# Stansfash/nonstationary-precip

Hardware: AMD Instinct MI355X
Metric: dsvi_elbo_steps_per_sec (higher is better)
Workload: dtype f32; 1 GPU; 2-layer DSVI DeepGP (hidden 3->2 + last 2->1), M=1024, S=10, minibatch 4096 (global, split over the GPUs) of synthetic N=1e5 spatio-temporal grid; fwd+ELBO+bwd+Adam; M=1024, S=10, per_gpu_batch=4096, global_batch=4096, N=100000, parallelism=dp1, kzz_cholesky_dtype=f64, hipgraph=True

## Files before the change

### nonstationary-precip_amd/csrc/gemm_i8.hip

```cpp
#include <cstdlib>
#include "common.h"

namespace {

#ifndef NSGP_I8_DMA
#define NSGP_I8_DMA 1
#endif
constexpr int I8_BM = 128, I8_BN = 64, I8_BK = 32;
constexpr int I8_SW = 5;

typedef int v4i __attribute__((ext_vector_type(4)));
typedef int v16i __attribute__((ext_vector_type(16)));

__global__ __launch_bounds__(256) void i8_slice_w_kernel(const double* __restrict__ W, int64_t M, int64_t Mp, int64_t KB,
                                                         signed char* __restrict__ Wd, double* __restrict__ wsc) {
    __shared__ double lds[4];
    const int64_t b = blockIdx.y, m = blockIdx.x;
    signed char* out = Wd + b * (int64_t)I8_SW * KB * 2 * Mp * 16;
    const int64_t plane = KB * 2 * Mp * 16;
    if (m >= M) {
        for (int64_t k = threadIdx.x; k < KB * 32; k += 256)
            for (int a = 0; a < I8_SW; ++a) out[a * plane + ((k >> 5) * 2 + ((k >> 4) & 1)) * Mp * 16 + m * 16 + (k & 15)] = 0;
        return;
    }
    const double* row = W + (b * M + m) * M;
    const auto nmax = [](double a, double c) { return (a > c || a != a) ? a : c; };
    double mx = 0.0;
    for (int64_t k = threadIdx.x; k <= m; k += 256) mx = nmax(fabs(row[k]), mx);
    for (int off = 32; off > 0; off >>= 1) mx = nmax(__shfl_xor(mx, off, 64), mx);
    if ((threadIdx.x & 63) == 0) lds[threadIdx.x >> 6] = mx;
    __syncthreads();
    mx = nmax(nmax(lds[0], lds[1]), nmax(lds[2], lds[3]));
    const bool fin = mx <= 1.7976931348623157e308;
    int e = 0;
    (void)frexp(fin ? mx : 0.0, &e);
    const double rs = (fin && mx > 0.0) ? ldexp(1.0, e) : 1.0;
    if (threadIdx.x == 0) wsc[b * M + m] = fin ? rs / 64.0 : __builtin_nan("");
    const double inv = 64.0 / rs;
    for (int64_t k = threadIdx.x; k < KB * 32; k += 256) {
        double t = (fin && k <= m && k < M) ? row[k] * inv : 0.0;
        const int64_t o = ((k >> 5) * 2 + ((k >> 4) & 1)) * Mp * 16 + m * 16 + (k & 15);
#pragma unroll
        for (int a = 0; a < I8_SW; ++a) {
            const double d = rint(t);
            out[a * plane + o] = (signed char)(int)d;
            t = (t - d) * 128.0;
        }
    }
}

template <int D, int SK>
__global__ __launch_bounds__(256) void i8_rbf_build_kernel(const float* __restrict__ Z, const float* __restrict__ x, int64_t sx,
                                                           const float* __restrict__ ls, const float* __restrict__ os,
                                                           int64_t M, int64_t n, int64_t np, int64_t KB,
                                                           signed char* __restrict__ Kd, double* __restrict__ ksc,
                                                           float* __restrict__ Kf) {
    const int64_t b = blockIdx.z, kb = blockIdx.y;
    const int64_t j = (int64_t)blockIdx.x * 256 + threadIdx.x;
    __shared__ double zs[32][D];
    __shared__ int bad;
    if (threadIdx.x == 0) bad = 0;
    if (threadIdx.x < 32 * D) {
        const int kk = threadIdx.x / D, d = threadIdx.x % D;
        const int64_t k = kb * 32 + kk;
        zs[kk][d] = k < M ? (double)Z[(b * M + k) * D + d] / (double)ls[b * D + d] : 0.0;
    }
    __syncthreads();
    const double osd = (double)os[b];
    bool fin = fabs(osd) <= 1.7976931348623157e308;
#pragma unroll
    for (int d = 0; d < D; ++d) fin = fin && fabs((double)ls[b * D + d]) <= 1.7976931348623157e308;
    int e = 0;
    (void)frexp(fin ? osd : 0.0, &e);
    const double cs = ldexp(1.0, e);
    const double sc = fin ? osd * 64.0 / cs : 0.0;
    if (j < np) {
        double xs[D];
#pragma unroll
        for (int d = 0; d < D; ++d) xs[d] = j < n ? (double)x[b * sx + j * D + d] / (double)ls[b * D + d] : 0.0;
        signed char* out = Kd + b * (int64_t)SK * KB * 2 * np * 16;
        const int64_t plane = KB * 2 * np * 16;
#pragma unroll
        for (int h = 0; h < 2; ++h) {
            int pk[SK][4] = {};
#pragma unroll
            for (int q = 0; q < 16; ++q) {
                const int kk = h * 16 + q;
                double r2 = 0.0;
#pragma unroll
                for (int d = 0; d < D; ++d) { const double df = zs[kk][d] - xs[d]; r2 = __builtin_fma(df, df, r2); }
                const bool in = j < n && kb * 32 + kk < M;
                const bool nan_e = in && r2 != r2;
                if (nan_e) bad = 1;
                const double ev = in ? t_fexp<double>(-0.5 * r2) : 0.0;
                const double evd = nan_e ? 0.0 : ev;
                if (Kf && in) Kf[(b * M + kb * 32 + kk) * n + j] = (float)(osd * ev);
                double t = sc * evd;
#pragma unroll
                for (int s = 0; s < SK; ++s) {
                    const double dg = rint(t);
                    pk[s][q >> 2] |= ((int)dg & 0xFF) << (8 * (q & 3));
                    t = (t - dg) * 128.0;
                }
            }
#pragma unroll
            for (int s = 0; s < SK; ++s) {
                v4i v = {pk[s][0], pk[s][1], pk[s][2], pk[s][3]};
                *reinterpret_cast<v4i*>(out + s * plane + (kb * 2 + h) * np * 16 + j * 16) = v;
            }
        }
    }
    __syncthreads();
    if (threadIdx.x == 0)
        ksc[(b * KB + kb) * gridDim.x + blockIdx.x] = (fin && !bad) ? cs / 64.0 : __builtin_nan("");
}

template <int P64, int SK, int LEV>
__global__ __launch_bounds__(256, 2) void i8_proj_kernel(const signed char* __restrict__ Wd, const double* __restrict__ wsc,
                                                         const signed char* __restrict__ Kd, const double* __restrict__ ksc,
                                                         const float* __restrict__ rv, int64_t M, int64_t n, int64_t Mp,
                                                         int64_t np, int64_t KB, int tiles_n, float* __restrict__ Y,
                                                         void* __restrict__ p0, void* __restrict__ p1, int part_rows) {
    extern __shared__ __attribute__((aligned(16))) unsigned char i8_smem[];
    constexpr int A_STAGE = I8_SW * 2 * I8_BM * 16, B_STAGE = SK * 2 * I8_BN * 16;
    unsigned char* As = i8_smem;
    unsigned char* Bs = i8_smem + 2 * A_STAGE;
    const int tid = threadIdx.x, lane = tid & 63, wave = __builtin_amdgcn_readfirstlane(tid >> 6);
    const int wm0 = (wave >> 1) * 64, wn0 = (wave & 1) * 32;
    const int64_t bb = blockIdx.y;
    const int tiles_m = (int)(Mp / I8_BM);
    const int bm = tiles_m - 1 - (int)blockIdx.x / tiles_n;
    const int bn = (int)blockIdx.x % tiles_n;
    const int64_t m0 = (int64_t)bm * I8_BM, n0 = (int64_t)bn * I8_BN;
    int nkb = (int)((m0 + I8_BM) / I8_BK);
    if (nkb > KB) nkb = (int)KB;
    const signed char* Wb = Wd + bb * (int64_t)I8_SW * KB * 2 * Mp * 16;
    const signed char* Kb = Kd + bb * (int64_t)SK * KB * 2 * np * 16;
    const int64_t wplane = KB * 2 * Mp * 16, kplane = KB * 2 * np * 16;

    const signed char* ga[5];
#pragma unroll
    for (int j = 0; j < 5; ++j) {
        const int q = tid + 256 * j;
        const int a = q >> 8, h = (q >> 7) & 1, row = q & 127;
        ga[j] = Wb + a * wplane + (int64_t)h * Mp * 16 + (m0 + row) * 16;
    }
    constexpr int NPB = (SK * 128 + 255) / 256;
    const signed char* gb[NPB];
#pragma unroll
    for (int j = 0; j < NPB; ++j) {
        int q = tid + 256 * j;
        if (q >= SK * 128) q = SK * 128 - 1;
        const int s = q >> 7, h = (q >> 6) & 1, col = q & 63;
        gb[j] = Kb + s * kplane + (int64_t)h * np * 16 + (n0 + col) * 16;
    }
    const int64_t astep = 2 * Mp * 16, bstep = 2 * np * 16;
#if NSGP_I8_DMA
    typedef const __attribute__((address_space(1))) void* gptr_t;
    typedef __attribute__((address_space(3))) void* lptr_t;
    auto dma = [&](int kb, int buf) __attribute__((always_inline)) {
#pragma unroll
        for (int j = 0; j < 5; ++j)
            __builtin_amdgcn_global_load_lds((gptr_t)(ga[j] + (int64_t)kb * astep),
                                             (lptr_t)(As + buf * A_STAGE + (wave * 64 + 256 * j) * 16), 16, 0, 0);
#pragma unroll
        for (int j = 0; j < NPB; ++j)
            if (wave * 64 + 256 * j < SK * 128)
                __builtin_amdgcn_global_load_lds((gptr_t)(gb[j] + (int64_t)kb * bstep),
                                                 (lptr_t)(Bs + buf * B_STAGE + (wave * 64 + 256 * j) * 16), 16, 0, 0);
    };
#endif
    v4i ra[5], rb[NPB];
    auto gload = [&](int kb) __attribute__((always_inline)) {
#pragma unroll
        for (int j = 0; j < 5; ++j) ra[j] = *reinterpret_cast<const v4i*>(ga[j] + (int64_t)kb * astep);
#pragma unroll
        for (int j = 0; j < NPB; ++j) rb[j] = *reinterpret_cast<const v4i*>(gb[j] + (int64_t)kb * bstep);
    };
    auto sstore = [&](int buf) __attribute__((always_inline)) {
#pragma unroll
        for (int j = 0; j < 5; ++j) *reinterpret_cast<v4i*>(As + buf * A_STAGE + (tid + 256 * j) * 16) = ra[j];
#pragma unroll
        for (int j = 0; j < NPB; ++j)
            if (tid + 256 * j < SK * 128) *reinterpret_cast<v4i*>(Bs + buf * B_STAGE + (tid + 256 * j) * 16) = rb[j];
    };

    v16i acc[LEV][2];
#pragma unroll
    for (int l = 0; l < LEV; ++l)
#pragma unroll
        for (int i = 0; i < 2; ++i)
#pragma unroll
            for (int r = 0; r < 16; ++r) acc[l][i][r] = 0;

    const int wave_nkb = __builtin_amdgcn_readfirstlane((int)((m0 + wm0 + 64 + I8_BK - 1) / I8_BK));
    const int half = lane >> 5, lr = lane & 31;
#if NSGP_I8_DMA
    dma(0, 0);
    asm volatile("s_waitcnt vmcnt(0)" ::: "memory");
#else
    gload(0);
    sstore(0);
#endif
    __syncthreads();
    for (int kb = 0; kb < nkb; ++kb) {
        const int buf = kb & 1;
#if NSGP_I8_DMA
        if (kb + 1 < nkb) dma(kb + 1, buf ^ 1);
#else
        if (kb + 1 < nkb) gload(kb + 1);
#endif
        if (kb < wave_nkb) {
            v4i af[2][2], bf[SK];
#pragma unroll
            for (int s = 0; s < SK; ++s)
                bf[s] = *reinterpret_cast<const v4i*>(Bs + buf * B_STAGE + ((s * 2 + half) * I8_BN + wn0 + lr) * 16);
#pragma unroll
            for (int i = 0; i < 2; ++i)
                af[0][i] = *reinterpret_cast<const v4i*>(As + buf * A_STAGE + ((0 * 2 + half) * I8_BM + wm0 + 32 * i + lr) * 16);
#pragma unroll
            for (int a = 0; a < I8_SW; ++a) {
                if (a + 1 < I8_SW) {
#pragma unroll
                    for (int i = 0; i < 2; ++i)
                        af[(a + 1) & 1][i] = *reinterpret_cast<const v4i*>(
                            As + buf * A_STAGE + (((a + 1) * 2 + half) * I8_BM + wm0 + 32 * i + lr) * 16);
                }
#pragma unroll
                for (int s = 0; s < SK; ++s)
                    if (a + s < LEV) {
#pragma unroll
                        for (int i = 0; i < 2; ++i)
                            acc[a + s][i] = __builtin_amdgcn_mfma_i32_32x32x32_i8(af[a & 1][i], bf[s], acc[a + s][i], 0, 0, 0);
                    }
            }
        }
#if NSGP_I8_DMA
        asm volatile("s_waitcnt vmcnt(0)" ::: "memory");
#else
        if (kb + 1 < nkb) sstore(buf ^ 1);
#endif
        __syncthreads();
    }

    const int64_t gx = (np + 255) >> 8;
    const double* ks = ksc + bb * KB * gx + (n0 >> 8);
    const double kslot = tid < nkb ? ks[(int64_t)tid * gx] : 0.0;
    const double kscale = __syncthreads_or(kslot != kslot) ? __builtin_nan("") : ks[0];
    double sdot = 0.0, ssq = 0.0;
    const int64_t col = n0 + wn0 + lr;
    const float* rvb = rv ? rv + bb * M : nullptr;
#pragma unroll
    for (int i = 0; i < 2; ++i)
#pragma unroll
        for (int r = 0; r < 16; ++r) {
            const int64_t row = m0 + wm0 + 32 * i + (r & 3) + 8 * (r >> 2) + 4 * half;
            double v = (double)acc[LEV - 1][i][r];
#pragma unroll
            for (int l = LEV - 2; l >= 0; --l) v = __builtin_fma(v, 0.0078125, (double)acc[l][i][r]);
            const bool in = row < M && col < n;
            v *= (in ? wsc[bb * M + row] : 0.0) * kscale;
            if (in) Y[(bb * M + row) * n + col] = (float)v;
            sdot += v * ((rvb && in) ? (double)rvb[row] : 0.0);
            ssq += v * v;
        }
    sdot += __shfl_xor(sdot, 32, 64);
    ssq += __shfl_xor(ssq, 32, 64);
    double* red = reinterpret_cast<double*>(i8_smem);
    __syncthreads();
    if (lane < 32) {
        red[(0 + (wave >> 1)) * I8_BN + wn0 + lane] = sdot;
        red[(2 + (wave >> 1)) * I8_BN + wn0 + lane] = ssq;
    }
    __syncthreads();
    if (tid < I8_BN && n0 + tid < n) {
        const int64_t o = (bb * part_rows + bm) * n + n0 + tid;
        const double d = red[tid] + red[I8_BN + tid], q = red[2 * I8_BN + tid] + red[3 * I8_BN + tid];
        if (P64) {
            if (p0) reinterpret_cast<double*>(p0)[o] = d;
            reinterpret_cast<double*>(p1)[o] = q;
        } else {
            if (p0) reinterpret_cast<float*>(p0)[o] = (float)d;
            reinterpret_cast<float*>(p1)[o] = (float)q;
        }
    }
}

static inline int64_t i8_mp(int64_t M) { return cdiv64(M, I8_BM) * I8_BM; }
static inline int64_t i8_np(int64_t n) { return cdiv64(n, I8_BN) * I8_BN; }
static inline int64_t i8_kb(int64_t M) { return cdiv64(M, I8_BK); }

}

extern "C" {

int nsgp_i8_supported(int64_t M) { return (M >= 1 && M <= 4096) ? 1 : 0; }
size_t nsgp_i8_w_planes_bytes(int64_t batch, int64_t M) {
    return (batch > 0 && M > 0) ? (size_t)(batch * I8_SW * i8_kb(M) * 2 * i8_mp(M) * 16) : 0;
}
size_t nsgp_i8_k_planes_bytes(int64_t batch, int64_t M, int64_t n, int planes) {
    return (batch > 0 && M > 0 && n > 0 && (planes == 4 || planes == 5)) ? (size_t)(batch * planes * i8_kb(M) * 2 * i8_np(n) * 16) : 0;
}
size_t nsgp_i8_tiles(int64_t M) { return M > 0 ? (size_t)cdiv64(M, I8_BM) : 0; }
size_t nsgp_i8_kscale_count(int64_t batch, int64_t M, int64_t n) {
    return (batch > 0 && M > 0 && n > 0) ? (size_t)(batch * i8_kb(M) * cdiv64(i8_np(n), 256)) : 0;
}

int nsgp_i8_slice_w_f64(const double* W, int64_t batch, int64_t M, void* Wd, double* wscale, void* stream) {
    if (!W) return -1; if (batch < 0) return -2; if (M < 0 || !nsgp_i8_supported(M > 0 ? M : 1)) return -3;
    if (!Wd) return -4; if (!wscale) return -5;
    if (batch == 0 || M == 0) return 0;
    if (batch > 65535) return -2;
    hipLaunchKernelGGL(i8_slice_w_kernel, dim3((unsigned)i8_mp(M), (unsigned)batch), dim3(256), 0, (hipStream_t)stream, W, M,
                       i8_mp(M), i8_kb(M), (signed char*)Wd, wscale);
    return nsgp_launch_status();
}

int nsgp_i8_rbf_build_f32(const float* Z, const float* x, int64_t x_batch_stride, const float* ls, const float* os,
                          int64_t batch, int64_t M, int64_t n, int D, int planes, void* Kd, double* kscale, float* Kzx_f32,
                          void* stream) {
    if (planes != 4 && planes != 5) return -10;
    if (!Z) return -1; if (!x) return -2; if (x_batch_stride < 0) return -3; if (!ls) return -4; if (!os) return -5;
    if (batch < 0) return -6; if (M < 0 || !nsgp_i8_supported(M > 0 ? M : 1)) return -7; if (n < 0) return -8;
    if (D < 1 || D > 4) return -9; if (!Kd) return -10; if (!kscale) return -11;
    if (batch == 0 || M == 0 || n == 0) return 0;
    if (batch > 65535 || i8_kb(M) > 65535) return -6;
    const int64_t np = i8_np(n), KB = i8_kb(M);
    dim3 grid((unsigned)cdiv64(np, 256), (unsigned)KB, (unsigned)batch);
    hipStream_t st = (hipStream_t)stream;
    signed char* kd = (signed char*)Kd;
#define NSGP_I8_BUILD(DD, SS) hipLaunchKernelGGL((i8_rbf_build_kernel<DD, SS>), grid, dim3(256), 0, st, Z, x, x_batch_stride, ls, os, M, n, np, KB, kd, kscale, Kzx_f32)
    if (planes == 4) {
        switch (D) { case 1: NSGP_I8_BUILD(1, 4); break; case 2: NSGP_I8_BUILD(2, 4); break; case 3: NSGP_I8_BUILD(3, 4); break;
                     default: NSGP_I8_BUILD(4, 4); break; }
    } else {
        switch (D) { case 1: NSGP_I8_BUILD(1, 5); break; case 2: NSGP_I8_BUILD(2, 5); break; case 3: NSGP_I8_BUILD(3, 5); break;
                     default: NSGP_I8_BUILD(4, 5); break; }
    }
#undef NSGP_I8_BUILD
    return nsgp_launch_status();
}

int nsgp_svgp_tri_gemm_colstats_i8(const void* Wd, const double* wscale, const void* Kd, const double* kscale,
                                   int planes, const float* rowvec, int64_t batch, int64_t M, int64_t n, float* Y,
                                   void* part_dot, void* part_sq, int64_t part_rows, int partials_f64, void* stream) {
    if (planes != 4 && planes != 5) return -5;
    if (!Wd) return -1; if (!wscale) return -2; if (!Kd) return -3; if (!kscale) return -4;
    if (batch < 0) return -6; if (M < 0 || !nsgp_i8_supported(M > 0 ? M : 1)) return -7; if (n < 0) return -8;
    if (!Y) return -9; if (!part_sq) return -11; if (part_rows < cdiv64(M > 0 ? M : 1, I8_BM)) return -12;
    if (batch == 0 || M == 0 || n == 0) return 0;
    const int64_t Mp = i8_mp(M), np = i8_np(n), KB = i8_kb(M);
    const int64_t tiles_n = np / I8_BN, tiles = (Mp / I8_BM) * tiles_n;
    if (tiles > 2147483647LL || batch > 65535) return -8;
    const size_t lds = 2 * (size_t)(I8_SW * 2 * I8_BM * 16 + planes * 2 * I8_BN * 16);
    hipStream_t st = (hipStream_t)stream;
    dim3 grid((unsigned)tiles, (unsigned)batch);
#define NSGP_I8_PROJ(PP, SS) hipLaunchKernelGGL((i8_proj_kernel<PP, SS, (SS == 5 ? 6 : 5)>), grid, dim3(256), lds, st, (const signed char*)Wd, wscale, \
        (const signed char*)Kd, kscale, rowvec, M, n, Mp, np, KB, (int)tiles_n, Y, part_dot, part_sq, (int)part_rows)
    if (planes == 4) { if (partials_f64) NSGP_I8_PROJ(1, 4); else NSGP_I8_PROJ(0, 4); }
    else { if (partials_f64) NSGP_I8_PROJ(1, 5); else NSGP_I8_PROJ(0, 5); }
#undef NSGP_I8_PROJ
    return nsgp_launch_status();
}

}
```

Baseline: 233.4 steps/s.

## Add persistent triple-buffered i8 projection kernel with wider tiles

Adds a persistent kernel for the triangular int8 projection GEMM. It launches one block per CU, walks tiles in a serpentine order starting from the heaviest triangular rows, doubles the N tile to 128 with 512 threads, and triple-buffers global-to-LDS DMA loads across tile boundaries. The aim is to cut launch and tail imbalance on the triangular workload and to overlap loads with MFMA. The old path stays reachable through an environment variable. It uses more LDS per block, and the occupancy and schedule are more complex.

```diff
diff --git a/nonstationary-precip_amd/csrc/gemm_i8.hip b/nonstationary-precip_amd/csrc/gemm_i8.hip
--- a/nonstationary-precip_amd/csrc/gemm_i8.hip
+++ b/nonstationary-precip_amd/csrc/gemm_i8.hip
@@ -1,3 +1,4 @@
+#include <atomic>
 #include <cstdlib>
 #include "common.h"
 
@@ -286,9 +287,188 @@
     }
 }
 
+template <int P64, int SK, int LEV>
+__global__ __launch_bounds__(512, 2) void i8_proj_persistent_kernel(
+        const signed char* __restrict__ Wd, const double* __restrict__ wsc, const signed char* __restrict__ Kd,
+        const double* __restrict__ ksc, const float* __restrict__ rv, int64_t M, int64_t n, int64_t Mp, int64_t np,
+        int64_t KB, int tiles_m, int tiles_n, int batch, float* __restrict__ Y, void* __restrict__ p0, void* __restrict__ p1,
+        int part_rows) {
+    extern __shared__ __attribute__((aligned(16))) unsigned char i8_smem[];
+    constexpr int BN = 2 * I8_BN;
+    constexpr int NL = 20 + 4 * SK;
+    constexpr int STAGE = NL * 1024;
+    constexpr int NJ = (NL + 7) / 8;
+    constexpr int NMIN = NL / 8;
+    double* red = reinterpret_cast<double*>(i8_smem + 3 * STAGE);
+    const int tid = threadIdx.x, lane = tid & 63, wave = __builtin_amdgcn_readfirstlane(tid >> 6);
+    const int wr = wave >> 2, wm0 = wr * 64, wn0 = (wave & 3) * 32;
+    const int half = lane >> 5, lr = lane & 31;
+    const int G = (int)gridDim.x, w = (int)blockIdx.x;
+    const int per_row = tiles_n * batch, T = tiles_m * per_row;
+    const int64_t wplane = KB * 2 * Mp * 16, kplane = KB * 2 * np * 16;
+    const int64_t astep = 2 * Mp * 16, bstep = 2 * np * 16;
+
+    const auto entry = [&](int r) { return r * G + ((r & 1) ? G - 1 - w : w); };
+    struct Tile { int bm, bb, bn, nkb; };
+    const auto tile_of = [&](int i) {
+        Tile t;
+        t.bm = tiles_m - 1 - i / per_row;
+        const int rem = i % per_row;
+        t.bb = rem / tiles_n;
+        t.bn = rem % tiles_n;
+        t.nkb = (int)((((int64_t)t.bm + 1) * I8_BM) / I8_BK);
+        if (t.nkb > KB) t.nkb = (int)KB;
+        return t;
+    };
+
+    typedef const __attribute__((address_space(1))) void* gptr_t;
+    typedef __attribute__((address_space(3))) void* lptr_t;
+    int pr = 0, pkb = 0;
+    Tile pt = tile_of(entry(0));
+    bool pmore = true;
+    const auto issue = [&](int buf) __attribute__((always_inline)) {
+        const int64_t m0 = (int64_t)pt.bm * I8_BM, n0 = (int64_t)pt.bn * BN;
+        const signed char* Wb = Wd + (int64_t)pt.bb * I8_SW * wplane + (int64_t)pkb * astep;
+        const signed char* Kb = Kd + (int64_t)pt.bb * SK * kplane + (int64_t)pkb * bstep;
+        const bool half_tile = n0 + I8_BN >= np;
+#pragma unroll
+        for (int j = 0; j < NJ; ++j) {
+            const int L = wave + 8 * j;
+            if (j < NMIN || L < NL) {
+                const signed char* src;
+                if (L < 20) {
+                    src = Wb + (L >> 2) * wplane + ((L >> 1) & 1) * Mp * 16 + (m0 + 64 * (L & 1) + lane) * 16;
+                } else {
+                    const int Lb = L - 20;
+                    const int c = half_tile ? 0 : (Lb & 1);
+                    src = Kb + (Lb >> 2) * kplane + ((Lb >> 1) & 1) * np * 16 + (n0 + 64 * c + lane) * 16;
+                }
+                __builtin_amdgcn_global_load_lds((gptr_t)src, (lptr_t)(i8_smem + buf * STAGE + L * 1024), 16, 0, 0);
+            }
+        }
+        if (++pkb == pt.nkb) {
+            pkb = 0;
+            const int i = entry(++pr);
+            pmore = i < T;
+            if (pmore) pt = tile_of(i);
+        }
+    };
+
+    int issued = 0;
+    issue(0);
+    ++issued;
+    if (pmore) { issue(1); ++issued; }
+    int g = 0, buf = 0;
+    for (int r = 0;; ++r) {
+        const int i = entry(r);
+        if (i >= T) break;
+        const Tile t = tile_of(i);
+        const int64_t m0 = (int64_t)t.bm * I8_BM, n0 = (int64_t)t.bn * BN;
+        v16i acc[LEV][2];
+#pragma unroll
+        for (int l = 0; l < LEV; ++l)
+#pragma unroll
+            for (int q = 0; q < 2; ++q)
+#pragma unroll
+                for (int e = 0; e < 16; ++e) acc[l][q][e] = 0;
+        const int wave_nkb = (int)((m0 + wm0 + 64 + I8_BK - 1) / I8_BK);
+        for (int kb = 0; kb < t.nkb; ++kb, ++g) {
+            if (issued > g + 1) asm volatile("s_waitcnt vmcnt(%0)" :: "n"(NMIN) : "memory");
+            else asm volatile("s_waitcnt vmcnt(0)" ::: "memory");
+            asm volatile("s_waitcnt lgkmcnt(0)" ::: "memory");
+            __builtin_amdgcn_s_barrier();
+            asm volatile("" ::: "memory");
+            if (pmore) { issue(buf == 0 ? 2 : buf - 1); ++issued; }
+            const unsigned char* As = i8_smem + buf * STAGE;
+            const unsigned char* Bs = As + I8_SW * 2 * I8_BM * 16;
+            if (kb < wave_nkb) {
+                v4i af[2][2], bf[SK];
+#pragma unroll
+                for (int s = 0; s < SK; ++s)
+                    bf[s] = *reinterpret_cast<const v4i*>(Bs + ((s * 2 + half) * BN + wn0 + lr) * 16);
+#pragma unroll
+                for (int q = 0; q < 2; ++q)
+                    af[0][q] = *reinterpret_cast<const v4i*>(As + ((0 * 2 + half) * I8_BM + wm0 + 32 * q + lr) * 16);
+#pragma unroll
+                for (int a = 0; a < I8_SW; ++a) {
+                    if (a + 1 < I8_SW) {
+#pragma unroll
+                        for (int q = 0; q < 2; ++q)
+                            af[(a + 1) & 1][q] = *reinterpret_cast<const v4i*>(
+                                As + (((a + 1) * 2 + half) * I8_BM + wm0 + 32 * q + lr) * 16);
+                    }
+#pragma unroll
+                    for (int s = 0; s < SK; ++s)
+                        if (a + s < LEV) {
+#pragma unroll
+                            for (int q = 0; q < 2; ++q)
+                                acc[a + s][q] = __builtin_amdgcn_mfma_i32_32x32x32_i8(af[a & 1][q], bf[s], acc[a + s][q], 0, 0, 0);
+                        }
+                }
+            }
+            buf = buf == 2 ? 0 : buf + 1;
+        }
+
+        const int64_t bb = t.bb;
+        const int64_t gx = (np + 255) >> 8;
+        const double* ks = ksc + bb * KB * gx + (n0 >> 8);
+        const double kslot = tid < t.nkb ? ks[(int64_t)tid * gx] : 0.0;
+        const double kscale = __syncthreads_or(kslot != kslot) ? __builtin_nan("") : ks[0];
+        double sdot = 0.0, ssq = 0.0;
+        const int64_t col = n0 + wn0 + lr;
+        const float* rvb = rv ? rv + bb * M : nullptr;
+#pragma unroll
+        for (int q = 0; q < 2; ++q)
+#pragma unroll
+            for (int e = 0; e < 16; ++e) {
+                const int64_t row = m0 + wm0 + 32 * q + (e & 3) + 8 * (e >> 2) + 4 * half;
+                double v = (double)acc[LEV - 1][q][e];
+#pragma unroll
+                for (int l = LEV - 2; l >= 0; --l) v = __builtin_fma(v, 0.0078125, (double)acc[l][q][e]);
+                const bool in = row < M && col < n;
+                const int64_t rowc = row < M ? row : M - 1;
+                const double ws = wsc[bb * M + rowc], rvv = rvb ? (double)rvb[rowc] : 0.0;
+                v *= (in ? ws : 0.0) * kscale;
+                if (in) Y[(bb * M + row) * n + col] = (float)v;
+                sdot += v * (in ? rvv : 0.0);
+                ssq += v * v;
+            }
+        sdot += __shfl_xor(sdot, 32, 64);
+        ssq += __shfl_xor(ssq, 32, 64);
+        if (lane < 32) {
+            red[(0 + wr) * BN + wn0 + lane] = sdot;
+            red[(2 + wr) * BN + wn0 + lane] = ssq;
+        }
+        __syncthreads();
+        if (tid < BN && n0 + tid < n) {
+            const int64_t o = (bb * part_rows + t.bm) * n + n0 + tid;
+            const double d = red[tid] + red[BN + tid], q = red[2 * BN + tid] + red[3 * BN + tid];
+            if (P64) {
+                if (p0) reinterpret_cast<double*>(p0)[o] = d;
+                reinterpret_cast<double*>(p1)[o] = q;
+            } else {
+                if (p0) reinterpret_cast<float*>(p0)[o] = (float)d;
+                reinterpret_cast<float*>(p1)[o] = (float)q;
+            }
+        }
+    }
+}
+
 static inline int64_t i8_mp(int64_t M) { return cdiv64(M, I8_BM) * I8_BM; }
 static inline int64_t i8_np(int64_t n) { return cdiv64(n, I8_BN) * I8_BN; }
 static inline int64_t i8_kb(int64_t M) { return cdiv64(M, I8_BK); }
+static int i8_cu_count() {
+    static std::atomic<int> cus[64];
+    int dev = 0;
+    (void)hipGetDevice(&dev);
+    std::atomic<int>& c = cus[dev & 63];
+    int v = c.load(std::memory_order_relaxed);
+    if (v <= 0) {
+        if (hipDeviceGetAttribute(&v, hipDeviceAttributeMultiprocessorCount, dev) != hipSuccess || v <= 0) v = 256;
+        c.store(v, std::memory_order_relaxed);
+    }
+    return v;
+}
 
 }
 
@@ -352,8 +532,25 @@
     const int64_t Mp = i8_mp(M), np = i8_np(n), KB = i8_kb(M);
     const int64_t tiles_n = np / I8_BN, tiles = (Mp / I8_BM) * tiles_n;
     if (tiles > 2147483647LL || batch > 65535) return -8;
+    hipStream_t st = (hipStream_t)stream;
+    const char* old = getenv("NSGP_I8_PROJ_OLD");
+    if (!(old && old[0] == '1')) {
+        const int64_t tiles_n2 = cdiv64(np, 2 * I8_BN), T = (Mp / I8_BM) * tiles_n2 * batch;
+        if (T > 2147483647LL) return -8;
+        const int G = (int)(T < i8_cu_count() ? T : i8_cu_count());
+        const size_t lds = 3 * (size_t)(20 + 4 * planes) * 1024 + 4 * 2 * I8_BN * sizeof(double);
+#define NSGP_I8_PERS(PP, SS) do { \
+            nsgp_opt_in_lds((const void*)i8_proj_persistent_kernel<PP, SS, (SS == 5 ? 6 : 5)>, lds); \
+            hipLaunchKernelGGL((i8_proj_persistent_kernel<PP, SS, (SS == 5 ? 6 : 5)>), dim3((unsigned)G), dim3(512), lds, st, \
+                               (const signed char*)Wd, wscale, (const signed char*)Kd, kscale, rowvec, M, n, Mp, np, KB, \
+                               (int)(Mp / I8_BM), (int)tiles_n2, (int)batch, Y, part_dot, part_sq, (int)part_rows); \
+        } while (0)
+        if (planes == 4) { if (partials_f64) NSGP_I8_PERS(1, 4); else NSGP_I8_PERS(0, 4); }
+        else { if (partials_f64) NSGP_I8_PERS(1, 5); else NSGP_I8_PERS(0, 5); }
+#undef NSGP_I8_PERS
+        return nsgp_launch_status();
+    }
     const size_t lds = 2 * (size_t)(I8_SW * 2 * I8_BM * 16 + planes * 2 * I8_BN * 16);
-    hipStream_t st = (hipStream_t)stream;
     dim3 grid((unsigned)tiles, (unsigned)batch);
 #define NSGP_I8_PROJ(PP, SS) hipLaunchKernelGGL((i8_proj_kernel<PP, SS, (SS == 5 ? 6 : 5)>), grid, dim3(256), lds, st, (const signed char*)Wd, wscale, \
         (const signed char*)Kd, kscale, rowvec, M, n, Mp, np, KB, (int)tiles_n, Y, part_dot, part_sq, (int)part_rows)
```

New measurement: 234.5 steps/s, median of 6. No clear change (+0.4%).
